# UnchartedWhispers/Distributed-Data-Parallel-Experiment

Measured on AMD Instinct MI355X. Metric: samples_per_sec_whole_node, higher is better.
Workload: dtype bf16

## Files before the change

csrc/include/ddpx_pipe.h:

```cpp
#pragma once

#include "ddpx_common.h"

namespace ddpx {
namespace pipe {

enum Epi : int {
  EPI_F32 = 0,
  EPI_BF16 = 1,
  EPI_BIAS_BF16 = 2,
  EPI_BIAS_RELU_BF16 = 3,
  EPI_BIAS_F32 = 4,
  EPI_RELUMASK_BF16 = 5,
  EPI_SGD = 6,
  EPI_BNSTAT_BF16 = 7,
  EPI_BNBWD_BF16 = 8,
};

enum Mode : int { MODE_PLAIN = 0, MODE_IM2COL_FWD = 1, MODE_IM2COL_BWD = 2, MODE_IM2COL_COL = 3 };

struct FastDiv {
  unsigned magic;
  int shift;
};
// ... 41 lines not shown
  int sgd_plain;
  float* slab;
  unsigned slab_bytes;
  int* tcnt;
  void* cs_out;
  int cs_flags;
  int* cs_tcnt;
  int im_slow;
  long long* stamp;
  const unsigned short* bn_y;
  const float* bn_a;
  const float* bn_b;
  const float* bn_mean;
  const float* bn_rstd;
  int bn_pool;
};

__device__ __forceinline__ void stamp_at(const Params& p, int tid, int k) {
  if (p.stamp && tid == 0)
    p.stamp[((size_t)blockIdx.y * gridDim.x + blockIdx.x) * 8 + k] = (long long)__builtin_amdgcn_s_memrealtime();
}

constexpr unsigned kOOB = 0x80000000u;

template <int ROWB>
__device__ __forceinline__ int tr_swz(int k) {
  if constexpr (ROWB >= 256) return (k & 3) | (((k >> 3) & 1) << 2);
  else if constexpr (ROWB == 128) return ((k >> 1) & 1) | (((k >> 3) & 1) << 1);
  else return (k >> 3) & 1;
}

// ... 253 lines not shown
  } else if constexpr (E == EPI_SGD) {
    stored = v * p.alpha;
    float d = fmaf(p.sgd.wd, pv, stored);
    if (p.sgd.mom != 0.f) {
      d = fmaf(p.sgd.mom, bv, d);
      *b_out = d;
    }
    *p_out = fmaf(-lr, d, pv);
  } else {
    const bool pos = (auxv & 0x8000u) == 0 && (auxv & 0x7fffu) != 0;
    stored = pos ? bf2f(f2bf(v * p.alpha)) : 0.f;
  }
  return stored;
}

template <int E, int BM, int BN, int NT = 256>
__device__ __forceinline__ void epilogue_vec(const Params& p, void* Cbase, const float* T, int m0, int n0, int tid,
                                             float (&csum)[4]) {
  constexpr int Q = BN / 4;
  constexpr int RSTEP = NT / Q;
  constexpr int NV = BM / RSTEP;
  constexpr int TLD = BN + 4;
  const int cq = tid % Q, r0 = tid / Q;
  const int n = n0 + 4 * cq;
  const bool vec = (n + 3 < p.N) && ((p.ldc & 3) == 0);
  float lr = 0.f;
  if constexpr (E == EPI_SGD) lr = *p.sgd.lr;
  constexpr bool HAS_BIAS = E == EPI_BIAS_BF16 || E == EPI_BIAS_RELU_BF16 || E == EPI_BIAS_F32;
  float bq[4] = {0.f, 0.f, 0.f, 0.f};
  if constexpr (HAS_BIAS) {
    if (vec && !(reinterpret_cast<uintptr_t>(p.bias + n) & 15)) {
      const f32x4 b4 = *reinterpret_cast<const f32x4*>(p.bias + n);
#pragma unroll
      for (int q = 0; q < 4; ++q) bq[q] = b4[q];
    } else {
#pragma unroll
      for (int q = 0; q < 4; ++q) bq[q] = n + q < p.N ? p.bias[n + q] : 0.f;
    }
  }
  constexpr int CH = E == EPI_SGD ? (NV < 8 ? NV : 8) : (NV < 4 ? NV : 4);
#pragma unroll
  for (int i0 = 0; i0 < NV; i0 += CH) {
  f32x4 pin[CH], bin[CH], cin[CH];
  u32x2 ain[CH];
#pragma unroll
  for (int i = 0; i < CH; ++i) {
    const int m = m0 + r0 + (i0 + i) * RSTEP;
    pin[i] = bin[i] = cin[i] = (f32x4){0.f, 0.f, 0.f, 0.f};
    ain[i] = (u32x2){0u, 0u};
    if (m >= p.M) continue;
    const size_t off = (size_t)m * p.ldc + n;
    if (vec) {
      if constexpr (E == EPI_SGD) {
        if (p.sgd_plain) {
          pin[i] = *reinterpret_cast<const f32x4*>(p.sgd.p + off);
          if (p.sgd.mom != 0.f) bin[i] = *reinterpret_cast<const f32x4*>(p.sgd.buf + off);
        } else {
          pin[i] = __builtin_nontemporal_load(reinterpret_cast<const f32x4*>(p.sgd.p + off));
          if (p.sgd.mom != 0.f) bin[i] = __builtin_nontemporal_load(reinterpret_cast<const f32x4*>(p.sgd.buf + off));
// ... 217 lines not shown
  const int kend = p.klen ? min(p.K, kbeg + p.klen) : p.K;
  void* Cbase = p.C;
  if (p.klen && !SK) Cbase = reinterpret_cast<char*>(p.C) + (size_t)split * p.split_stride * (p.epi == EPI_F32 ? 4 : 2);

  const __amdgpu_buffer_rsrc_t ra = __builtin_amdgcn_make_buffer_rsrc((void*)p.A, 0, p.a_bytes, 0x00020000);
  const __amdgpu_buffer_rsrc_t rb = __builtin_amdgcn_make_buffer_rsrc((void*)p.B, 0, p.b_bytes, 0x00020000);

  f32x4 acc[FM][FN];
#pragma unroll
  for (int i = 0; i < FM; ++i)
#pragma unroll
    for (int j = 0; j < FN; ++j) acc[i][j] = (f32x4){0.f, 0.f, 0.f, 0.f};

  const int nk = (kend - kbeg + BK - 1) / BK;

  constexpr bool A_IM = AK && (AMODE == MODE_IM2COL_FWD || AMODE == MODE_IM2COL_BWD);
  ImRows<A_IM ? BM : 8 * NW, NW> arow;
  const bool a_fast = A_IM && !p.im_slow && (p.conv.C & 63) == 0;
  if constexpr (A_IM) {
    if (a_fast) im_rows_init<BM, NW>(arow, p.conv, m0, p.M, wave, lane);
  }
  constexpr bool B_COL = !BKc && BMODE == MODE_IM2COL_COL;
  ColRows<B_COL ? BN : 8 * NW, NW> bcol;
  const bool b_fast = B_COL && !p.im_slow && (64 % p.conv.W) == 0;
  if constexpr (B_COL) {
    if (b_fast) col_rows_init<BN, NW>(bcol, p.conv, n0, p.N, wave, lane);
  }

  auto issue = [&](int t) {
    char* slot = smem + (t % STAGES) * SLOT;
// ... 55 lines not shown
      }
      for (int j = nk > D ? nk - D : 0; j < nk; ++j) {
        wait_vmcnt_rt((nk - 1 - j) * LPL);
        lds_signal(ring_full + j % STAGES, lane);
      }
      return;
    }
    for (int t = 0; t < nk; ++t) {
      const int sl = t % STAGES;
      lds_wait_ge(ring_full + sl, (t / STAGES + 1) * LW);
      mma_slot(t);
      asm volatile("s_waitcnt lgkmcnt(0)" ::: "memory");
      lds_signal(ring_free + sl, lane);
    }
  } else {
#pragma unroll
  for (int s = 0; s < STAGES - 1; ++s)
    if (s < nk) issue(s);

  for (int t = 0; t < nk; ++t) {
    const int ahead = min(STAGES - 2, nk - 1 - t);
    if (STAGES >= 6 && ahead >= 4) wait_vmcnt<(STAGES >= 6 ? 4 : 0) * LPW>();
    else if (STAGES >= 5 && ahead >= 3) wait_vmcnt<(STAGES >= 5 ? 3 : 0) * LPW>();
    else if (ahead >= 2) wait_vmcnt<2 * LPW>();
    else if (ahead == 1) wait_vmcnt<LPW>();
    else wait_vmcnt<0>();
    __builtin_amdgcn_s_barrier();
    asm volatile("" ::: "memory");
    if (t + STAGES - 1 < nk) issue(t + STAGES - 1);
    mma_slot(t);
// ... 30 lines not shown
        for (int j = 0; j < FN; ++j)
          v[i][j] = __builtin_bit_cast(f32x4, __builtin_amdgcn_raw_buffer_load_b128(rsl, slab_off(sp, i * FN + j), 0,
                                                                                    16 ));
#pragma unroll
      for (int i = 0; i < FM; ++i)
#pragma unroll
        for (int j = 0; j < FN; ++j) acc[i][j] = sp == 0 ? v[i][j] : acc[i][j] + v[i][j];
    }
    stamp_at(p, tid, 3);
  }

  constexpr int TLD = BN + 4;
  constexpr int SCR = (NT / (BN / 4) + 2) * BN * 4;
  constexpr int EH = (BM * TLD * 4 + SCR <= STAGES * SLOT) ? 1 : ((BM / 2) * TLD * 4 + SCR <= STAGES * SLOT) ? 2 : 4;
  static_assert(WGM % EH == 0, "epilogue parts must align with wave rows");
  constexpr int BMH = BM / EH;
  constexpr int WPH = WGM / EH;
  float* T = reinterpret_cast<float*>(smem);
  static_assert(BMH * TLD * 4 + SCR <= STAGES * SLOT, "epilogue LDS overflow");
  float* red = T + BMH * TLD;
  float* colres = red + (NT / (BN / 4)) * BN;
  float cs[4] = {0.f, 0.f, 0.f, 0.f};
  float st_n = 0.f, st_mean = 0.f, st_m2 = 0.f;
#pragma unroll
  for (int h = 0; h < EH; ++h) {
    if (h == 0) __builtin_amdgcn_s_barrier();
    else __syncthreads();
    if (wm / WPH == h) {
      const int mr = (wm % WPH) * (BM / WGM) + 4 * (lane >> 4);
      const int nc = wn * (BN / 2) + (lane & 15);
// ... 23 lines not shown
        if constexpr (LW == 0 && AMODE == MODE_IM2COL_BWD &&
                      ((NW == 8 && BM == 256 && BN == 128 && STAGES == 3) ||
                       (NW == 8 && BM == 128 && BN == 128 && STAGES != 3))) {
          float s2[4] = {0.f, 0.f, 0.f, 0.f};
          epilogue_bnbwd<BMH, BN, NT>(p, Cbase, T, mh, n0, tid, ch, s2);
          __syncthreads();
          quad_colsum<BN, NT>(red, ch, tid, colres);
          const size_t st = (size_t)tm * EH + h;
          if (tid < BN && n0 + tid < p.N) p.colsum[(st * 2) * p.N + n0 + tid] = colres[tid];
          quad_colsum<BN, NT>(red, s2, tid, colres);
          if (tid < BN && n0 + tid < p.N) p.colsum[(st * 2 + 1) * p.N + n0 + tid] = colres[tid];
#pragma unroll
          for (int q = 0; q < 4; ++q) ch[q] = 0.f;
        }
        break;
      default: epilogue_vec<EPI_RELUMASK_BF16, BMH, BN, NT>(p, Cbase, T, mh, n0, tid, ch); break;
    }
#pragma unroll
    for (int q = 0; q < 4; ++q) cs[q] += ch[q];
    if (LW == 0 && p.colsum && p.epi == EPI_BNSTAT_BF16) {
      __syncthreads();
      quad_colsum<BN, NT>(red, ch, tid, colres);
      const int rows_valid = min(BMH, p.M - mh);
      float* tmean = colres + BN;
      if (tid < BN) tmean[tid] = rows_valid > 0 ? colres[tid] / (float)rows_valid : 0.f;
      __syncthreads();
      {
        constexpr int Q = BN / 4, RSTEP = NT / Q, NV = BMH / RSTEP;
        const int cq = tid % Q, r0 = tid / Q;
        float m2[4] = {0.f, 0.f, 0.f, 0.f};
#pragma unroll
// ... 67 lines not shown
      v[q] = __uint_as_float(__builtin_amdgcn_raw_buffer_load_b32(
          rcs, (unsigned)(((size_t)(t0 + q) * p.N + n0 + tid) * 4), 0, 16 ));
#pragma unroll
    for (int q = 0; q < 8; ++q) tot += v[q];
  }
  const int n = n0 + tid;
  if (p.sgd.p) {
    sgd_apply_pre(p.sgd, n, tot, lrv, pv, mv);
  } else if (p.cs_flags & 1) {
    unsigned short* o = reinterpret_cast<unsigned short*>(p.cs_out) + n;
    *o = f2bf((p.cs_flags & 2) ? tot + bf2f(*o) : tot);
  } else {
    float* o = reinterpret_cast<float*>(p.cs_out) + n;
    *o = (p.cs_flags & 2) ? tot + *o : tot;
  }
}

template <int BM, int BN, int STAGES, bool AK, bool BKc, int AMODE, int BMODE, int NW = 4, int KSUB = 1,
          bool SK = false, int LW = 0>
static hipError_t launch(const Params& p, int splits, hipStream_t s) {
  const int tiles = ((p.M + BM - 1) / BM) * ((p.N + BN - 1) / BN);
  hipLaunchKernelGGL((gemm_pipe_kernel<BM, BN, STAGES, AK, BKc, AMODE, BMODE, NW, KSUB, SK, LW>),
                     dim3(tiles, splits), dim3((NW + LW) * 64), 0, s, p);
  return hipGetLastError();
}

constexpr int kNumCfgs = 26;
static inline bool eight_wave(int cfg) {
  return cfg == 8 || cfg == 13 || cfg == 14 || cfg == 15 || cfg == 22 || cfg == 25;
}
// ... 79 lines not shown
```

csrc/include/ddpx_wgrad_sgd.h:

```cpp
#pragma once

#include <cstdlib>

#include "ddpx_mx.h"
#include "ddpx_pipe.h"

namespace ddpx {
namespace wsgd {

constexpr int BN = 128;
constexpr int NK = 8;
constexpr int kStampSlots = 256;

template <int BM, int STAGES>
struct Cfg {
  static_assert(BM == 64 || BM == 128, "tile height");
  static_assert(STAGES == 3 || (STAGES == 4 && BM == 64), "ring depth");
  static constexpr int A_SUB = BM * 64 * 2, B_SUB = BN * 64 * 2, SLOT = A_SUB + B_SUB;
  static constexpr bool SBUF = BM == 128;
  static constexpr int ALD = (STAGES >= 4 || SBUF) ? BN : BN + 4;
  static constexpr int ACC_BYTES = BM * ALD * 4;
  static constexpr int LDS_BYTES = STAGES * SLOT + (SBUF ? 1 : 2) * ACC_BYTES;
  static_assert(LDS_BYTES <= 160 * 1024, "LDS");
  __host__ __device__ static constexpr int tile_col(int row, int col) {
    return SBUF ? (col ^ (((row >> 2) & 3) << 4)) : col;
  }
};

template <int BM, int STAGES, bool FP8, int NSW, bool NORD, int NMW, int PROBE = 0>
__global__ void __launch_bounds__(64 * NMW + 64 * NSW) wgrad_sgd_ws_kernel(pipe::Params p0, pipe::Params p1, int nt1) {
  using C = Cfg<BM, STAGES>;
  constexpr int ALD = C::ALD, ACC_BYTES = C::ACC_BYTES, LDS_BYTES = C::LDS_BYTES;
  constexpr int A_SUB = C::A_SUB, SLOT = C::SLOT;
  constexpr bool SBUF = C::SBUF;
  static_assert(NMW == 4 || NMW == 8, "math waves");
  static_assert(BM == 64 || (NMW == 8 && !FP8), "the 128-row tile: 8 math waves, no MX-FP8 copy");
  static_assert(PROBE == 0 || PROBE == 3 || PROBE == 4, "probe");
  constexpr int WN = NMW / 2;
  constexpr int WMR = BM / 2;
  constexpr int FM = WMR / 16, FN = BN / WN / 16;
  constexpr int LPW = (BM + BN) / (8 * NMW);
  __shared__ __attribute__((aligned(1024))) char smem[LDS_BYTES];
  float* const accb = reinterpret_cast<float*>(smem + STAGES * SLOT);

  const int tid = threadIdx.x;
// ... 215 lines not shown
      const float inv = ldexpf(1.f, -e);
      const unsigned lo = mx::quant4(v[0], v[1], v[2], v[3], inv, mx::kMaxE4M3, false);
      const unsigned hi = mx::quant4(v[4], v[5], v[6], v[7], inv, mx::kMaxE4M3, false);
      const int Mg = sel ? p1.M : p0.M;
      *reinterpret_cast<u32x2*>(qd + (size_t)(n0 + c) * Mg + m0 + 32 * b + 8 * sub) = (u32x2){lo, hi};
      unsigned char* const ed = sel ? ET1 : ET0;
      if (sub == 0 && ed) {
        if (b == 0) {
          qt_e0 = (unsigned)(e + 127);
        } else {
          *reinterpret_cast<unsigned short*>(ed + (size_t)(n0 + c) * (Mg / 32) + m0 / 32) =
              (unsigned short)(qt_e0 | ((unsigned)(e + 127) << 8));
        }
      }
    };
#pragma unroll
    for (int v = 0; v < DIST; ++v)
      if constexpr (PROBE != 3) load_vec(0, v, rp[v], rm[v]);
    for (int t = 0; t < nk; ++t) {
      mark();
      __builtin_amdgcn_s_barrier();
    }
    mark();
    __builtin_amdgcn_s_barrier();
    constexpr int TPI = SV / DIST;
    f32x4 gq[UPK];
    auto read_ahead = [&](int v0) {
      if constexpr (SBUF && PROBE != 3) {
#pragma unroll
        for (int k = 0; k < UPK; ++k) gq[k] = grad_vec(accb, v0 + k);
// ... 88 lines not shown
  Variant v;
  v.bm = 64;
  v.stages = (env_stages == 3 || env_stages == 4) ? env_stages : (large ? 4 : 3);
  v.fp8 = fp8;
  v.nsw = qt ? 8 : (env_nsw == 4 || env_nsw == 8) ? env_nsw : (large ? 8 : 4);
  v.nord = env_nord;
  v.nmw = (env_nmw != 4 && v.nsw == 4 && v.nord) ? 8 : 4;
  const bool can128 = m128 && !fp8 && !qt && env_stages != 4 && env_nsw != 8 && env_nmw != 4 && env_nord;
  const bool want128 = env_tile == 128 || (env_tile != 64 && ntiles >= 2LL * num_cus);
  if (want128 && can128) v.bm = 128, v.stages = 3, v.nsw = 4, v.nmw = 8;
  const bool toy = !fp8 && v.stages == 3 && v.nsw == 4 && v.nord;
  v.probe = (toy && (env_probe == 3 || env_probe == 4)) ? env_probe : 0;
  return v;
}

using Kernel = void (*)(pipe::Params, pipe::Params, int);

template <int STAGES, bool FP8>
static inline Kernel layout_kernel(const Variant& v) {
  if (v.nmw == 8) return wgrad_sgd_ws_kernel<64, STAGES, FP8, 4, true, 8>;
  if (v.nsw == 8) return v.nord ? wgrad_sgd_ws_kernel<64, STAGES, FP8, 8, true, 4>
                                : wgrad_sgd_ws_kernel<64, STAGES, FP8, 8, false, 4>;
  return v.nord ? wgrad_sgd_ws_kernel<64, STAGES, FP8, 4, true, 4> : wgrad_sgd_ws_kernel<64, STAGES, FP8, 4, false, 4>;
}

static inline Kernel kernel_of(const Variant& v) {
  if (v.bm == 128) {
    if (v.probe == 3) return wgrad_sgd_ws_kernel<128, 3, false, 4, true, 8, 3>;
    if (v.probe == 4) return wgrad_sgd_ws_kernel<128, 3, false, 4, true, 8, 4>;
    return wgrad_sgd_ws_kernel<128, 3, false, 4, true, 8>;
  }
  if (v.probe == 3)
    return v.nmw == 8 ? wgrad_sgd_ws_kernel<64, 3, false, 4, true, 8, 3> : wgrad_sgd_ws_kernel<64, 3, false, 4, true, 4, 3>;
  if (v.probe == 4)
    return v.nmw == 8 ? wgrad_sgd_ws_kernel<64, 3, false, 4, true, 8, 4> : wgrad_sgd_ws_kernel<64, 3, false, 4, true, 4, 4>;
  if (v.stages == 4) return v.fp8 ? layout_kernel<4, true>(v) : layout_kernel<4, false>(v);
  return v.fp8 ? layout_kernel<3, true>(v) : layout_kernel<3, false>(v);
}

static inline Variant plan(const pipe::Params& p0, const pipe::Params& p1, bool pair, bool qt, int num_cus) {
  const long long nt64 = (long long)(p0.M / 64) * (p0.N / BN) + (pair ? (long long)(p1.M / 64) * (p1.N / BN) : 0);
  const bool m128 = p0.M % 128 == 0 && (!pair || p1.M % 128 == 0);
  return select_variant(nt64, num_cus, p0.sgd.q8 != nullptr, qt, m128);
}

static inline hipError_t launch_variant(const pipe::Params& p0, const pipe::Params& p1, bool pair, bool qt,
                                        int num_cus, hipStream_t s) {
  const Variant v = plan(p0, p1, pair, qt, num_cus);
  const int nt1 = pair ? (p1.M / v.bm) * (p1.N / BN) : 0;
  const int ntiles = (p0.M / v.bm) * (p0.N / BN) + nt1;
  const int grid = ntiles < num_cus ? ntiles : num_cus;
  hipLaunchKernelGGL(kernel_of(v), dim3(grid), dim3(64 * (v.nmw + v.nsw)), 0, s, p0, p1, nt1);
  return hipGetLastError();
}

static inline hipError_t launch(const pipe::Params& p, int num_cus, hipStream_t s) {
  return launch_variant(p, p, false, false, num_cus, s);
}

static inline bool pair_compatible(const pipe::Params& a, const pipe::Params& b) {
  return a.K == b.K && a.alpha == b.alpha && a.sgd.lr == b.sgd.lr && a.sgd.mom == b.sgd.mom && a.sgd.wd == b.sgd.wd;
}

static inline hipError_t launch_pair(const pipe::Params& p0, const pipe::Params& p1, int num_cus, hipStream_t s) {
  if ((p0.sgd.q8 != nullptr) != (p1.sgd.q8 != nullptr)) return hipErrorInvalidValue;
  const bool qt = p0.sgd.q8t != nullptr || p1.sgd.q8t != nullptr;
  if (qt && !p0.sgd.q8) return hipErrorInvalidValue;
  return launch_variant(p0, p1, true, qt, num_cus, s);
}

}
}
```

csrc/kernels/gemm_pipe.hip:

```cpp
#include <cstdlib>

#include "ddpx_gemm_dispatch.h"
#include "ddpx_pipe.h"
#include "ddpx_wgrad_sgd.h"

namespace ddpx {
namespace pipe {

static int pick(int M, int N, int K, bool ak, bool bk) {
  auto tiles = [&](int bm, int bn) { return ((M + bm - 1) / bm) * ((N + bn - 1) / bn); };
  if (!ak && !bk) return tiles(64, 128) >= 512 ? 5 : 7;
  if (tiles(128, 128) >= 512 && K >= 2048) return 21;
  return 12;
}

static int plan(int M, int N, int K, bool ak, bool bk, int epi, int* cfg) {
  *cfg = pick(M, N, K, ak, bk);
  static const int sk_cfg = [] {
    const char* e = getenv("DDPX_SPLITK");
    return e ? atoi(e) : 0;
  }();
  static const int sk_max = [] {
    const char* e = getenv("DDPX_SPLITK_MAX");
    return e ? atoi(e) : 2;
// ... 57 lines not shown
  if (a_bytes >= 0x80000000ull || b_bytes >= 0x80000000ull) return -4;
  pipe::Params p{(const unsigned short*)A, (const unsigned short*)B, C, bias, (const unsigned short*)aux, colsum,
                 M, N, K, lda, ldb, ldc, ldaux, epi, accumulate, alpha, (unsigned)a_bytes, (unsigned)b_bytes,
                 SgdArgs{sgd_p, sgd_buf, (unsigned short*)sgd_shadow, sgd_lr, sgd_mom, sgd_wd},
                 pipe::make_geom(0, 0, 0, 0), 0, 0, 0, nullptr, 0u, nullptr, cs_out, cs_flags, cs_tcnt};
  p.stamp = g_stamp;
  if (cs_tcnt && (!colsum || epi == pipe::EPI_SGD || epi == pipe::EPI_BNSTAT_BF16 || (!cs_out && !sgd_p) ||
                  (sgd_p && !sgd_lr)))
    return -10;
  if (epi == pipe::EPI_SGD && (!sgd_p || !sgd_lr || (sgd_mom != 0.f && !sgd_buf))) return -5;
  static const int sgd_plain = [] {
    const char* e = getenv("DDPX_SGD_PLAIN");
    return e && e[0] == '1' ? 1 : 0;
  }();
  p.sgd_plain = sgd_plain;
  int cfg = tile_cfg >= 0 ? tile_cfg : pipe::pick(M, N, K, a_kcontig, b_kcontig);
  if (cs_tcnt && pipe::eight_wave(cfg)) return -11;
  if (cfg >= 16 && cfg <= 20 && (epi == pipe::EPI_SGD || epi == pipe::EPI_BNSTAT_BF16)) return -12;
  if (splits > 1) {
    if (epi == pipe::EPI_SGD || epi == pipe::EPI_BNSTAT_BF16 || !slab || !tcnt || tile_cfg < 0 || !a_kcontig)
      return -7;
    int bm, bn;
    pipe::tile_of(cfg, &bm, &bn);
    const long long tiles = (long long)((M + bm - 1) / bm) * ((N + bn - 1) / bn);
    if (slab_floats < (long long)splits * tiles * bm * bn || slab_floats * 4 >= 0x80000000ll) return -8;
    int klen = (K + splits - 1) / splits;
    klen = (klen + 63) / 64 * 64;
    if ((K + klen - 1) / klen != splits) return -9;
    p.klen = klen;
    p.slab = slab;
// ... 18 lines not shown
    return (int)wsgd::launch(p, cus, stream);
  }
  hipError_t e;
  if (splits > 1) {
    e = b_kcontig ? pipe::dispatch_sk_kk(p, cfg, splits, stream) : pipe::dispatch_sk_kn(p, cfg, splits, stream);
    return (int)e;
  }
  const int S = 1;
  if (a_kcontig && b_kcontig) e = pipe::dispatch_kk(p, cfg, S, stream);
  else if (a_kcontig) e = pipe::dispatch_kn(p, cfg, S, stream);
  else if (b_kcontig) e = pipe::dispatch_mk(p, cfg, S, stream);
  else e = pipe::dispatch_mn(p, cfg, S, stream);
  return (int)e;
}

DDPX_API int ddpx_wgrad_sgd_pair_t(const void* A0, const void* B0, int M0, int N0, int lda0, int ldb0, int ldc0,
                                   float* p0, float* buf0, void* sh0, void* q80, void* s80, void* q8t0, void* s8t0,
                                   const void* A1, const void* B1, int M1, int N1, int lda1, int ldb1, int ldc1,
                                   float* p1, float* buf1, void* sh1, void* q81, void* s81, void* q8t1, void* s8t1,
                                   int K, const float* lr, float mom, float wd, hipStream_t stream) {
  auto make = [&](const void* A, const void* B, int M, int N, int lda, int ldb, int ldc, float* pp, float* buf,
                  void* sh, void* q8, void* s8, void* q8t, void* s8t) {
    const size_t a_bytes = ((size_t)(K - 1) * lda + M) * 2, b_bytes = ((size_t)(K - 1) * ldb + N) * 2;
    return pipe::Params{(const unsigned short*)A, (const unsigned short*)B, pp, nullptr, nullptr, nullptr,
                        M, N, K, lda, ldb, ldc, 0, pipe::EPI_SGD, 0, 1.f, (unsigned)a_bytes, (unsigned)b_bytes,
                        SgdArgs{pp, buf, (unsigned short*)sh, lr, mom, wd, (unsigned char*)q8, (unsigned char*)s8,
                                (unsigned char*)q8t, (unsigned char*)s8t},
                        pipe::make_geom(0, 0, 0, 0), 0, 0, 0, nullptr, 0u, nullptr, nullptr, 0, nullptr};
  };
  if (K <= 0 || lda0 % 8 || ldb0 % 8 || lda1 % 8 || ldb1 % 8 || M0 % 8 || N0 % 8 || M1 % 8 || N1 % 8) return -20;
  if (((uintptr_t)A0 | (uintptr_t)B0 | (uintptr_t)A1 | (uintptr_t)B1) & 15) return -20;
  if ((q8t0 || q8t1) && (!q80 || !q81)) return -20;
  pipe::Params q0 = make(A0, B0, M0, N0, lda0, ldb0, ldc0, p0, buf0, sh0, q80, s80, q8t0, s8t0);
  const pipe::Params q1 = make(A1, B1, M1, N1, lda1, ldb1, ldc1, p1, buf1, sh1, q81, s81, q8t1, s8t1);
  q0.stamp = g_stamp;
  if ((size_t)q0.a_bytes != ((size_t)(K - 1) * lda0 + M0) * 2 || (size_t)q1.b_bytes != ((size_t)(K - 1) * ldb1 + N1) * 2)
    return -20;
  if (!wsgd::eligible(q0, false, false) || !wsgd::eligible(q1, false, false) || !wsgd::pair_compatible(q0, q1))
    return -20;
  if ((q80 != nullptr) != (q81 != nullptr)) return -20;
  int dev = 0, cus = 0;
  if (hipGetDevice(&dev) != hipSuccess ||
      hipDeviceGetAttribute(&cus, hipDeviceAttributeMultiprocessorCount, dev) != hipSuccess || cus <= 0)
    cus = 256;
  return (int)wsgd::launch_pair(q0, q1, cus, stream);
}

DDPX_API int ddpx_wgrad_sgd_pair(const void* A0, const void* B0, int M0, int N0, int lda0, int ldb0, int ldc0,
                                 float* p0, float* buf0, void* sh0, void* q80, void* s80, const void* A1,
                                 const void* B1, int M1, int N1, int lda1, int ldb1, int ldc1, float* p1, float* buf1,
                                 void* sh1, void* q81, void* s81, int K, const float* lr, float mom, float wd,
                                 hipStream_t stream) {
  return ddpx_wgrad_sgd_pair_t(A0, B0, M0, N0, lda0, ldb0, ldc0, p0, buf0, sh0, q80, s80, nullptr, nullptr, A1, B1,
                               M1, N1, lda1, ldb1, ldc1, p1, buf1, sh1, q81, s81, nullptr, nullptr, K, lr, mom, wd,
                               stream);
}

DDPX_API int ddpx_wgrad_sgd_plan(int M0, int N0, int M1, int N1, int K, int fp8, int qt, int* bm, int* stages,
                                 int* nsw, int* nmw) {
  const bool pair = M1 > 0;
// ... 19 lines not shown
```

ddpx/ops/gemm.py:

```python
from __future__ import annotations

import torch

from ..runtime import native


EPI_F32 = 0
EPI_BF16 = 1
EPI_BIAS_BF16 = 2
EPI_BIAS_RELU_BF16 = 3
EPI_BIAS_F32 = 4
EPI_RELUMASK_BF16 = 5
EPI_SGD = 6

_OUT_DTYPE = {
    EPI_F32: torch.float32,
    EPI_BF16: torch.bfloat16,
    EPI_BIAS_BF16: torch.bfloat16,
    EPI_BIAS_RELU_BF16: torch.bfloat16,
    EPI_BIAS_F32: torch.float32,
    EPI_RELUMASK_BF16: torch.bfloat16,
}


# ... 93 lines not shown
    if out_dtype == torch.bfloat16:
        epi = EPI_BIAS_RELU_BF16 if relu else (EPI_BIAS_BF16 if bias is not None else EPI_BF16)
        _req(not (relu and bias is None), "relu epilogue requires a bias")
    else:
        _req(not relu, "fp32 output epilogue has no relu")
        epi = EPI_BIAS_F32 if bias is not None else EPI_F32
    if out is None:
        out = torch.empty((M, N), dtype=_OUT_DTYPE[epi], device=x.device)
    _req(tuple(out.shape) == (M, N) and out.stride(1) == 1 and out.stride(0) % 8 == 0
         and out.data_ptr() % 16 == 0 and out.dtype == _OUT_DTYPE[epi], "bad out tensor")
    return gemm_raw(x, w, out, M=M, N=N, K=K, lda=x.stride(0), ldb=w.stride(0), ldc=out.stride(0), a_kcontig=True,
                    b_kcontig=True, epi=epi, bias=bias, tile=tile, splits=splits)


def linear_dgrad(dy, w, relu_mask_of=None, out=None, tile=-1, bias_grad=None, bias_grad_accumulate=False,
                 bias_sgd=None, splits=None):
    _check_bf16_2d(dy, "dy")
    _check_bf16_2d(w, "w")
    M, N = dy.shape
    N2, K = w.shape
    _req(N == N2, f"dy {tuple(dy.shape)} incompatible with w {tuple(w.shape)}")
    epi = EPI_BF16
    if relu_mask_of is not None:
        _check_bf16_2d(relu_mask_of, "relu_mask_of")
        _req(tuple(relu_mask_of.shape) == (M, K), "mask shape must equal dX shape")
        epi = EPI_RELUMASK_BF16
    if out is None:
        out = torch.empty((M, K), dtype=torch.bfloat16, device=dy.device)
    _req(out.shape == (M, K) and out.is_contiguous() and out.dtype == torch.bfloat16, "bad out tensor")
    part = None
    if bias_grad is not None or bias_sgd is not None:
        _req(bias_grad is None or (bias_grad.numel() == K and bias_grad.is_contiguous()),
             "bias_grad must be contiguous [K]")
        _req(bias_sgd is None or bias_sgd[0].numel() == K, "bias_sgd target must have K elements")
        T = tiles_m(M, K, N, True, False, tile)
        part = torch.empty((T, K), dtype=torch.float32, device=dy.device)
    in_launch = tile not in _EIGHT_WAVE_TILES
    _req(in_launch or bias_sgd is None, "fused bias SGD needs a 4-wave dgrad tile")
    gemm_raw(dy, w, out, M=M, N=K, K=N, lda=dy.stride(0), ldb=w.stride(0), ldc=K, a_kcontig=True,
             b_kcontig=False, epi=epi, aux=relu_mask_of,
             ldaux=(relu_mask_of.stride(0) if relu_mask_of is not None else 0), tile=tile, colsum=part,
             splits=splits,
             cs_out=bias_grad if in_launch else None, cs_accumulate=bias_grad_accumulate,
             cs_sgd=bias_sgd if in_launch else None)
    if part is not None and not in_launch and bias_grad is not None:
        s = part.sum(0).to(bias_grad.dtype)
        bias_grad.add_(s) if bias_grad_accumulate else bias_grad.copy_(s)
    return out


_EIGHT_WAVE_TILES = (8, 13, 14, 15, 22, 25)

# ... 32 lines not shown


native.register_kernel_sig("ddpx_wgrad_sgd_pair", native.c_int, *([native.c_void_p, native.c_void_p] + [native.c_int] * 5
                                                                  + [native.c_void_p] * 5) * 2,
                           native.c_int, native.c_void_p, native.c_float, native.c_float, native.c_void_p)


native.register_kernel_sig("ddpx_wgrad_sgd_pair_t", native.c_int, *([native.c_void_p, native.c_void_p] + [native.c_int] * 5
                                                                    + [native.c_void_p] * 7) * 2,
                           native.c_int, native.c_void_p, native.c_float, native.c_float, native.c_void_p)


native.register_kernel_sig("ddpx_wgrad_sgd_plan", native.c_int, *([native.c_int] * 7 + [native.c_void_p] * 4))


def wgrad_sgd_plan(M0, N0, M1=0, N1=0, K=512, fp8=False, transposed=False):
    import ctypes
    out = [ctypes.c_int(0) for _ in range(4)]
    rc = native.kernels().ddpx_wgrad_sgd_plan(int(M0), int(N0), int(M1), int(N1), int(K), int(bool(fp8)),
                                              int(bool(transposed)), *[ctypes.addressof(o) for o in out])
    if rc == -20:
        return None
    native.check(rc, "ddpx_wgrad_sgd_plan")
    return dict(zip(("bm", "stages", "nsw", "nmw"), (o.value for o in out)))


def wgrad_sgd_pair(dy0, x0, sgd0, dy1, x1, sgd1, mx0=None, mx1=None, mxt0=None, mxt1=None) -> bool:
    for t, n in ((dy0, "dy0"), (x0, "x0"), (dy1, "dy1"), (x1, "x1")):
        _check_bf16_2d(t, n)
    if dy0.shape[0] != dy1.shape[0] or x0.shape[0] != dy0.shape[0] or x1.shape[0] != dy1.shape[0]:
        return False
    if sgd0[3] is not sgd1[3] or sgd0[4] != sgd1[4] or sgd0[5] != sgd1[5]:
        return False
    K = dy0.shape[0]
    transposed = mxt0 is not None or mxt1 is not None
    if transposed and (mx0 is None or mx1 is None):
        return False
    args = []
    for dy, x, sg, mx, mxt in ((dy0, x0, sgd0, mx0, mxt0), (dy1, x1, sgd1, mx1, mxt1)):
        M, N = dy.shape[1], x.shape[1]
        _req(sg[0].numel() == M * N, "sgd target size mismatch")
        if mx is not None:
            _req(mx[0].dtype == torch.uint8 and mx[0].numel() == M * N and mx[0].is_contiguous()
                 and mx[1].dtype == torch.uint8 and mx[1].numel() == M * N // 32 and N % 32 == 0,
                 "fp8 copy must be uint8 [M, N] codes + [M, N/32] scales")
        if mxt is not None:
            _req(mxt[0].dtype == torch.uint8 and tuple(mxt[0].shape) == (N, M) and mxt[0].is_contiguous()
                 and mxt[1].dtype == torch.uint8 and tuple(mxt[1].shape) == (N, M // 32) and mxt[1].is_contiguous()
                 and M % 64 == 0, "transposed fp8 copy must be uint8 [N, M] codes + [N, M/32] scales, M % 64 == 0")
        args += [dy.data_ptr(), x.data_ptr(), M, N, dy.stride(0), x.stride(0), N, sg[0].data_ptr(),
                 native.ptr(sg[1]), native.ptr(sg[2]), native.ptr(mx[0] if mx else None),
                 native.ptr(mx[1] if mx else None)]
        if transposed:
            args += [native.ptr(mxt[0] if mxt else None), native.ptr(mxt[1] if mxt else None)]
    lr = sg[3]
    fn = native.kernels().ddpx_wgrad_sgd_pair_t if transposed else native.kernels().ddpx_wgrad_sgd_pair
    rc = fn(*args, K, lr.data_ptr(), float(sgd0[4]), float(sgd0[5]), native.stream_handle())
    if rc == -20:
        return False
    native.check(rc, "ddpx_wgrad_sgd_pair")
    return True
```

ddpx/ops/mlp.py:

```python
from __future__ import annotations

import os

import torch

from . import gemm as G
from ..optim.sgd import take_lr_advance
from .head import head_backward, head_forward

_PAIR_WGRAD = os.environ.get("DDPX_WGRAD_PAIR", "1") != "0"
_FP8_WGRAD = os.environ.get("DDPX_FP8_WGRAD", "0") == "1"
_FP8_DGRAD = os.environ.get("DDPX_FP8_DGRAD", "0") == "1"


def _dgrad_mx8(dpre, wq, h, bias_grad=None, bias_acc=False, bias_sgd=None):
    from . import fp8 as F8
    from .elementwise import colsum_bf16, sgd_flat_
    dq = F8.quant(dpre, F8.E4M3)
    dx = F8.gemm(dq, wq, epi=G.EPI_RELUMASK_BF16, aux=h)
    if bias_sgd is not None:
        p, buf, sh, lr, mom, wd = bias_sgd
        g = torch.empty(p.numel(), dtype=torch.float32, device=dx.device)
        colsum_bf16(dx, g)
        sgd_flat_(p, buf if buf is not None else torch.zeros_like(p), g, sh, lr, mom, wd)
    elif bias_grad is not None:
        if bias_grad.dtype == torch.float32:
            colsum_bf16(dx, bias_grad, accumulate=bias_acc)
# ... 81 lines not shown
    ps = _params(model)
    L = len(ps) - 1
    wl, bl = ps[-1]
    bprev = ps[L - 1][1]
    fused = flat.fused_spec(wl) is not None
    fp8_dgrad = _FP8_DGRAD and bool(getattr(model, "fp8", False)) and hs[L].is_cuda
    if fp8_dgrad and flat.shadow8t is None and not torch.cuda.is_current_stream_capturing():
        flat.enable_fp8_transposed()
    dpre = torch.empty_like(hs[L])
    if fused:
        head_backward(dl, grad_out, hs[L], flat.shadow_of(wl), None, None, dH=dpre, relu_mask=True,
                      sgd_w=flat.fused_spec(wl), sgd_b=flat.fused_spec(bl), sgd_prev=flat.fused_spec(bprev))
        for p in (wl, bl, bprev):
            flat.mark_updated(p)
        deferred = None
        for l in range(L - 1, -1, -1):
            w, _ = ps[l]
            dnext = None
            if l > 0:
                bp = ps[l - 1][1]
                if fp8_dgrad:
                    dnext = _dgrad_mx8(dpre, flat.mx8t_weight(w), hs[l], bias_sgd=flat.fused_spec(bp))
                else:
                    dnext = G.linear_dgrad(dpre, flat.shadow_of(w), relu_mask_of=hs[l], bias_sgd=flat.fused_spec(bp))
                flat.mark_updated(bp)
            if l == 1 and not saved8 and _PAIR_WGRAD:
                deferred = (dpre, hs[1], flat.fused_spec(w), w)
            elif l == 0 and deferred is not None:
                d1, h1, s1, w1 = deferred
                s0 = flat.fused_spec(w)
                emit = flat.shadow8 is not None and flat.fp8_from_optimizer
                mx1, mx0 = (flat.mx8_views(w1), flat.mx8_views(w)) if emit else (None, None)
                if mx1 is None or mx0 is None:
                    mx1 = mx0 = None
                mxt1 = flat.mx8t_views(w1) if (fp8_dgrad and mx1 is not None) else None
                paired = G.wgrad_sgd_pair(d1, h1, s1, dpre, hs[0], s0, mx1, mx0, mxt1, None)
                if not paired:
                    G.linear_wgrad(d1, h1, None, sgd=s1)
                    _wgrad(saved8, 0, dpre, hs[0], None, sgd=s0)
                flat.mark_updated(w1, fp8_written=paired and mx1 is not None,
                                  fp8t_written=paired and mxt1 is not None)
                flat.mark_updated(w, fp8_written=paired and mx0 is not None)
                dpre = dnext
                continue
            else:
                _wgrad(saved8, l, dpre, hs[l], None, sgd=flat.fused_spec(w))
            flat.mark_updated(w)
            dpre = dnext
        return
    dW, acc = flat.grad_target(wl)
    db, accb = flat.grad_target(bl)
    dbp, accp = flat.grad_target(bprev)
# ... 84 lines not shown
```

Before: 2.465 million.

## Defer dgrad bias colsum-SGD into paired wgrad kernel and prefetch relu mask

The layer-1 dgrad no longer finishes its bias column-sum and SGD update inside its own launch. It writes per-tile partials, and the paired wgrad+SGD kernel reduces them and applies the bias update in its producer warps, with a standalone finish kernel as fallback. Separately, the 64x64 two-stage plain GEMM tile now issues the relu-mask aux loads for the epilogue before the main K loop so their latency overlaps compute. This is meant to remove a serialized in-launch finish step and hide epilogue load latency, at the cost of extra registers and more work placed in the wgrad kernel.

```diff
diff --git a/csrc/include/ddpx_pipe.h b/csrc/include/ddpx_pipe.h
--- a/csrc/include/ddpx_pipe.h
+++ b/csrc/include/ddpx_pipe.h
@@ -79,7 +79,18 @@
   const float* bn_mean;
   const float* bn_rstd;
   int bn_pool;
+  int epi_pf;
 };
+
+struct EpiPre {
+  u32x4 lo, hi;
+};
+
+template <int BM, int BN, int STAGES, int AMODE, int BMODE, int NW, int KSUB, bool SK, int LW>
+constexpr bool epi_prefetch_tile() {
+  return BM == 64 && BN == 64 && STAGES == 2 && NW == 4 && KSUB == 2 && !SK && LW == 0 && AMODE == MODE_PLAIN &&
+         BMODE == MODE_PLAIN;
+}
 
 __device__ __forceinline__ void stamp_at(const Params& p, int tid, int k) {
   if (p.stamp && tid == 0)
@@ -363,9 +374,33 @@
   return stored;
 }
 
-template <int E, int BM, int BN, int NT = 256>
+template <int BM, int BN, int NT>
+__device__ __forceinline__ EpiPre epi_prefetch(const Params& p, int m0, int n0, int tid) {
+  constexpr int Q = BN / 4, RSTEP = NT / Q, NV = BM / RSTEP;
+  static_assert(NV <= 4, "the prefetch holds one chunk of 4 vectors");
+  const int cq = tid % Q, r0 = tid / Q;
+  const int n = n0 + 4 * cq;
+  const bool vec = (n + 3 < p.N) && ((p.ldc & 3) == 0);
+  EpiPre pre{(u32x4){0u, 0u, 0u, 0u}, (u32x4){0u, 0u, 0u, 0u}};
+  if (p.epi == EPI_RELUMASK_BF16) {
+    if (vec) {
+      u32x2 a[4] = {{0u, 0u}, {0u, 0u}, {0u, 0u}, {0u, 0u}};
+#pragma unroll
+      for (int i = 0; i < NV; ++i) {
+        const int m = m0 + r0 + i * RSTEP;
+        a[i] = *reinterpret_cast<const u32x2*>(p.aux + (m < p.M ? (size_t)m * p.ldaux : (size_t)0) + n);
+      }
+      pre.lo = (u32x4){a[0][0], a[0][1], a[1][0], a[1][1]};
+      pre.hi = (u32x4){a[2][0], a[2][1], a[3][0], a[3][1]};
+    }
+  }
+  return pre;
+}
+
+template <int E, int BM, int BN, int NT = 256, bool PF = false>
 __device__ __forceinline__ void epilogue_vec(const Params& p, void* Cbase, const float* T, int m0, int n0, int tid,
-                                             float (&csum)[4]) {
+                                             float (&csum)[4], const EpiPre pre = EpiPre{},
+                                             bool use_pre = false) {
   constexpr int Q = BN / 4;
   constexpr int RSTEP = NT / Q;
   constexpr int NV = BM / RSTEP;
@@ -392,6 +427,19 @@
   for (int i0 = 0; i0 < NV; i0 += CH) {
   f32x4 pin[CH], bin[CH], cin[CH];
   u32x2 ain[CH];
+  bool loaded = false;
+  if constexpr (PF && E == EPI_RELUMASK_BF16) {
+    if (use_pre && i0 == 0) {
+      loaded = true;
+#pragma unroll
+      for (int i = 0; i < CH; ++i) {
+        pin[i] = bin[i] = cin[i] = (f32x4){0.f, 0.f, 0.f, 0.f};
+        const u32x4 h = i < 2 ? pre.lo : pre.hi;
+        ain[i] = (i & 1) ? (u32x2){h[2], h[3]} : (u32x2){h[0], h[1]};
+      }
+    }
+  }
+  if (!loaded)
 #pragma unroll
   for (int i = 0; i < CH; ++i) {
     const int m = m0 + r0 + (i0 + i) * RSTEP;
@@ -639,6 +687,10 @@
 
   const int nk = (kend - kbeg + BK - 1) / BK;
 
+  constexpr bool PF = epi_prefetch_tile<BM, BN, STAGES, AMODE, BMODE, NW, KSUB, SK, LW>();
+  EpiPre epf{(u32x4){0u, 0u, 0u, 0u}, (u32x4){0u, 0u, 0u, 0u}};
+  const bool use_pre = PF && p.epi_pf;
+
   constexpr bool A_IM = AK && (AMODE == MODE_IM2COL_FWD || AMODE == MODE_IM2COL_BWD);
   ImRows<A_IM ? BM : 8 * NW, NW> arow;
   const bool a_fast = A_IM && !p.im_slow && (p.conv.C & 63) == 0;
@@ -724,6 +776,9 @@
       lds_signal(ring_free + sl, lane);
     }
   } else {
+  if constexpr (PF) {
+    if (use_pre) epf = epi_prefetch<BM, BN, NT>(p, m0, n0, tid);
+  }
 #pragma unroll
   for (int s = 0; s < STAGES - 1; ++s)
     if (s < nk) issue(s);
@@ -784,6 +839,7 @@
   constexpr int SCR = (NT / (BN / 4) + 2) * BN * 4;
   constexpr int EH = (BM * TLD * 4 + SCR <= STAGES * SLOT) ? 1 : ((BM / 2) * TLD * 4 + SCR <= STAGES * SLOT) ? 2 : 4;
   static_assert(WGM % EH == 0, "epilogue parts must align with wave rows");
+  static_assert(!PF || EH == 1, "the prefetched chunk is the first chunk of the whole tile");
   constexpr int BMH = BM / EH;
   constexpr int WPH = WGM / EH;
   float* T = reinterpret_cast<float*>(smem);
@@ -837,7 +893,7 @@
           for (int q = 0; q < 4; ++q) ch[q] = 0.f;
         }
         break;
-      default: epilogue_vec<EPI_RELUMASK_BF16, BMH, BN, NT>(p, Cbase, T, mh, n0, tid, ch); break;
+      default: epilogue_vec<EPI_RELUMASK_BF16, BMH, BN, NT, PF>(p, Cbase, T, mh, n0, tid, ch, epf, use_pre); break;
     }
 #pragma unroll
     for (int q = 0; q < 4; ++q) cs[q] += ch[q];
@@ -935,6 +991,37 @@
     float* o = reinterpret_cast<float*>(p.cs_out) + n;
     *o = (p.cs_flags & 2) ? tot + *o : tot;
   }
+}
+
+struct ColFinish {
+  const float* part;
+  int tiles_m, n;
+  SgdArgs sgd;
+};
+
+__device__ __forceinline__ void colsum_finish_col(const ColFinish& cf, int n) {
+  const __amdgpu_buffer_rsrc_t rcs = __builtin_amdgcn_make_buffer_rsrc(
+      (void*)cf.part, 0, (unsigned)((size_t)cf.tiles_m * cf.n * 4), 0x00020000);
+  const float pv = __builtin_nontemporal_load(cf.sgd.p + n);
+  float mv = 0.f;
+  if (cf.sgd.mom != 0.f) mv = __builtin_nontemporal_load(cf.sgd.buf + n);
+  const float lrv = *cf.sgd.lr;
+  float tot = 0.f;
+  for (int t0 = 0; t0 < cf.tiles_m; t0 += 8) {
+    float v[8];
+#pragma unroll
+    for (int q = 0; q < 8; ++q)
+      v[q] = __uint_as_float(
+          __builtin_amdgcn_raw_buffer_load_b32(rcs, (unsigned)(((size_t)(t0 + q) * cf.n + n) * 4), 0, 0));
+#pragma unroll
+    for (int q = 0; q < 8; ++q) tot += v[q];
+  }
+  sgd_apply_pre(cf.sgd, n, tot, lrv, pv, mv);
+}
+
+static inline bool colfinish_ok(const ColFinish& cf) {
+  return cf.part && cf.tiles_m > 0 && cf.n > 0 && (size_t)cf.tiles_m * cf.n * 4 < 0x80000000ull && cf.sgd.p &&
+         cf.sgd.lr && (cf.sgd.mom == 0.f || cf.sgd.buf);
 }
 
 template <int BM, int BN, int STAGES, bool AK, bool BKc, int AMODE, int BMODE, int NW = 4, int KSUB = 1,
diff --git a/csrc/include/ddpx_wgrad_sgd.h b/csrc/include/ddpx_wgrad_sgd.h
--- a/csrc/include/ddpx_wgrad_sgd.h
+++ b/csrc/include/ddpx_wgrad_sgd.h
@@ -28,7 +28,8 @@
 };
 
 template <int BM, int STAGES, bool FP8, int NSW, bool NORD, int NMW, int PROBE = 0>
-__global__ void __launch_bounds__(64 * NMW + 64 * NSW) wgrad_sgd_ws_kernel(pipe::Params p0, pipe::Params p1, int nt1) {
+__global__ void __launch_bounds__(64 * NMW + 64 * NSW)
+wgrad_sgd_ws_kernel(pipe::Params p0, pipe::Params p1, int nt1, pipe::ColFinish cf) {
   using C = Cfg<BM, STAGES>;
   constexpr int ALD = C::ALD, ACC_BYTES = C::ACC_BYTES, LDS_BYTES = C::LDS_BYTES;
   constexpr int A_SUB = C::A_SUB, SLOT = C::SLOT;
@@ -274,6 +275,10 @@
         }
       }
     };
+    if (cf.part) {
+      for (int c0 = 16 * (int)blockIdx.x; c0 < cf.n; c0 += 16 * (int)gridDim.x)
+        if (st < 16 && c0 + st < cf.n) pipe::colsum_finish_col(cf, c0 + st);
+    }
 #pragma unroll
     for (int v = 0; v < DIST; ++v)
       if constexpr (PROBE != 3) load_vec(0, v, rp[v], rm[v]);
@@ -392,7 +397,7 @@
   return v;
 }
 
-using Kernel = void (*)(pipe::Params, pipe::Params, int);
+using Kernel = void (*)(pipe::Params, pipe::Params, int, pipe::ColFinish);
 
 template <int STAGES, bool FP8>
 static inline Kernel layout_kernel(const Variant& v) {
@@ -423,12 +428,12 @@
 }
 
 static inline hipError_t launch_variant(const pipe::Params& p0, const pipe::Params& p1, bool pair, bool qt,
-                                        int num_cus, hipStream_t s) {
+                                        int num_cus, hipStream_t s, const pipe::ColFinish& cf = pipe::ColFinish{}) {
   const Variant v = plan(p0, p1, pair, qt, num_cus);
   const int nt1 = pair ? (p1.M / v.bm) * (p1.N / BN) : 0;
   const int ntiles = (p0.M / v.bm) * (p0.N / BN) + nt1;
   const int grid = ntiles < num_cus ? ntiles : num_cus;
-  hipLaunchKernelGGL(kernel_of(v), dim3(grid), dim3(64 * (v.nmw + v.nsw)), 0, s, p0, p1, nt1);
+  hipLaunchKernelGGL(kernel_of(v), dim3(grid), dim3(64 * (v.nmw + v.nsw)), 0, s, p0, p1, nt1, cf);
   return hipGetLastError();
 }
 
@@ -440,12 +445,13 @@
   return a.K == b.K && a.alpha == b.alpha && a.sgd.lr == b.sgd.lr && a.sgd.mom == b.sgd.mom && a.sgd.wd == b.sgd.wd;
 }
 
-static inline hipError_t launch_pair(const pipe::Params& p0, const pipe::Params& p1, int num_cus, hipStream_t s) {
+static inline hipError_t launch_pair(const pipe::Params& p0, const pipe::Params& p1, int num_cus, hipStream_t s,
+                                     const pipe::ColFinish& cf = pipe::ColFinish{}) {
   if ((p0.sgd.q8 != nullptr) != (p1.sgd.q8 != nullptr)) return hipErrorInvalidValue;
   const bool qt = p0.sgd.q8t != nullptr || p1.sgd.q8t != nullptr;
   if (qt && !p0.sgd.q8) return hipErrorInvalidValue;
-  return launch_variant(p0, p1, true, qt, num_cus, s);
-}
-
-}
-}
+  return launch_variant(p0, p1, true, qt, num_cus, s, cf);
+}
+
+}
+}
diff --git a/csrc/kernels/gemm_pipe.hip b/csrc/kernels/gemm_pipe.hip
--- a/csrc/kernels/gemm_pipe.hip
+++ b/csrc/kernels/gemm_pipe.hip
@@ -95,6 +95,11 @@
     return e && e[0] == '1' ? 1 : 0;
   }();
   p.sgd_plain = sgd_plain;
+  static const int epi_pf = [] {
+    const char* e = getenv("DDPX_EPI_PREFETCH");
+    return e && e[0] == '0' ? 0 : 1;
+  }();
+  p.epi_pf = epi_pf;
   int cfg = tile_cfg >= 0 ? tile_cfg : pipe::pick(M, N, K, a_kcontig, b_kcontig);
   if (cs_tcnt && pipe::eight_wave(cfg)) return -11;
   if (cfg >= 16 && cfg <= 20 && (epi == pipe::EPI_SGD || epi == pipe::EPI_BNSTAT_BF16)) return -12;
@@ -143,11 +148,12 @@
   return (int)e;
 }
 
-DDPX_API int ddpx_wgrad_sgd_pair_t(const void* A0, const void* B0, int M0, int N0, int lda0, int ldb0, int ldc0,
-                                   float* p0, float* buf0, void* sh0, void* q80, void* s80, void* q8t0, void* s8t0,
-                                   const void* A1, const void* B1, int M1, int N1, int lda1, int ldb1, int ldc1,
-                                   float* p1, float* buf1, void* sh1, void* q81, void* s81, void* q8t1, void* s8t1,
-                                   int K, const float* lr, float mom, float wd, hipStream_t stream) {
+static int wgrad_sgd_pair_impl(const void* A0, const void* B0, int M0, int N0, int lda0, int ldb0, int ldc0,
+                               float* p0, float* buf0, void* sh0, void* q80, void* s80, void* q8t0, void* s8t0,
+                               const void* A1, const void* B1, int M1, int N1, int lda1, int ldb1, int ldc1,
+                               float* p1, float* buf1, void* sh1, void* q81, void* s81, void* q8t1, void* s8t1,
+                               int K, const float* lr, float mom, float wd, const pipe::ColFinish& cf,
+                               hipStream_t stream) {
   auto make = [&](const void* A, const void* B, int M, int N, int lda, int ldb, int ldc, float* pp, float* buf,
                   void* sh, void* q8, void* s8, void* q8t, void* s8t) {
     const size_t a_bytes = ((size_t)(K - 1) * lda + M) * 2, b_bytes = ((size_t)(K - 1) * ldb + N) * 2;
@@ -172,7 +178,43 @@
   if (hipGetDevice(&dev) != hipSuccess ||
       hipDeviceGetAttribute(&cus, hipDeviceAttributeMultiprocessorCount, dev) != hipSuccess || cus <= 0)
     cus = 256;
-  return (int)wsgd::launch_pair(q0, q1, cus, stream);
+  return (int)wsgd::launch_pair(q0, q1, cus, stream, cf);
+}
+
+DDPX_API int ddpx_wgrad_sgd_pair_t(const void* A0, const void* B0, int M0, int N0, int lda0, int ldb0, int ldc0,
+                                   float* p0, float* buf0, void* sh0, void* q80, void* s80, void* q8t0, void* s8t0,
+                                   const void* A1, const void* B1, int M1, int N1, int lda1, int ldb1, int ldc1,
+                                   float* p1, float* buf1, void* sh1, void* q81, void* s81, void* q8t1, void* s8t1,
+                                   int K, const float* lr, float mom, float wd, hipStream_t stream) {
+  return wgrad_sgd_pair_impl(A0, B0, M0, N0, lda0, ldb0, ldc0, p0, buf0, sh0, q80, s80, q8t0, s8t0, A1, B1, M1, N1,
+                             lda1, ldb1, ldc1, p1, buf1, sh1, q81, s81, q8t1, s8t1, K, lr, mom, wd, pipe::ColFinish{},
+                             stream);
+}
+
+DDPX_API int ddpx_wgrad_sgd_pair_cs(const void* A0, const void* B0, int M0, int N0, int lda0, int ldb0, int ldc0,
+                                    float* p0, float* buf0, void* sh0, void* q80, void* s80, void* q8t0, void* s8t0,
+                                    const void* A1, const void* B1, int M1, int N1, int lda1, int ldb1, int ldc1,
+                                    float* p1, float* buf1, void* sh1, void* q81, void* s81, void* q8t1, void* s8t1,
+                                    int K, const float* lr, float mom, float wd, const float* cs_part, int cs_tiles_m,
+                                    int cs_n, float* cs_p, float* cs_buf, void* cs_sh, const float* cs_lr, float cs_mom,
+                                    float cs_wd, hipStream_t stream) {
+  const pipe::ColFinish cf{cs_part, cs_tiles_m, cs_n, SgdArgs{cs_p, cs_buf, (unsigned short*)cs_sh, cs_lr, cs_mom, cs_wd}};
+  if (!pipe::colfinish_ok(cf)) return -21;
+  return wgrad_sgd_pair_impl(A0, B0, M0, N0, lda0, ldb0, ldc0, p0, buf0, sh0, q80, s80, q8t0, s8t0, A1, B1, M1, N1,
+                             lda1, ldb1, ldc1, p1, buf1, sh1, q81, s81, q8t1, s8t1, K, lr, mom, wd, cf, stream);
+}
+
+__global__ void __launch_bounds__(64) dgrad_colsum_finish_kernel(pipe::ColFinish cf) {
+  const int n = blockIdx.x * 64 + threadIdx.x;
+  if (n < cf.n) pipe::colsum_finish_col(cf, n);
+}
+
+DDPX_API int ddpx_dgrad_colsum_finish(const float* cs_part, int cs_tiles_m, int cs_n, float* cs_p, float* cs_buf,
+                                void* cs_sh, const float* cs_lr, float cs_mom, float cs_wd, hipStream_t stream) {
+  const pipe::ColFinish cf{cs_part, cs_tiles_m, cs_n, SgdArgs{cs_p, cs_buf, (unsigned short*)cs_sh, cs_lr, cs_mom, cs_wd}};
+  if (!pipe::colfinish_ok(cf)) return -21;
+  hipLaunchKernelGGL(dgrad_colsum_finish_kernel, dim3((cs_n + 63) / 64), dim3(64), 0, stream, cf);
+  return (int)hipGetLastError();
 }
 
 DDPX_API int ddpx_wgrad_sgd_pair(const void* A0, const void* B0, int M0, int N0, int lda0, int ldb0, int ldc0,
diff --git a/ddpx/ops/gemm.py b/ddpx/ops/gemm.py
--- a/ddpx/ops/gemm.py
+++ b/ddpx/ops/gemm.py
@@ -131,7 +131,7 @@
 
 
 def linear_dgrad(dy, w, relu_mask_of=None, out=None, tile=-1, bias_grad=None, bias_grad_accumulate=False,
-                 bias_sgd=None, splits=None):
+                 bias_sgd=None, splits=None, defer_finish=False):
     _check_bf16_2d(dy, "dy")
     _check_bf16_2d(w, "w")
     M, N = dy.shape
@@ -153,6 +153,13 @@
         T = tiles_m(M, K, N, True, False, tile)
         part = torch.empty((T, K), dtype=torch.float32, device=dy.device)
     in_launch = tile not in _EIGHT_WAVE_TILES
+    if defer_finish:
+        _req(bias_sgd is not None and bias_grad is None, "defer_finish needs bias_sgd (and no bias_grad)")
+        gemm_raw(dy, w, out, M=M, N=K, K=N, lda=dy.stride(0), ldb=w.stride(0), ldc=K, a_kcontig=True,
+                 b_kcontig=False, epi=epi, aux=relu_mask_of,
+                 ldaux=(relu_mask_of.stride(0) if relu_mask_of is not None else 0), tile=tile, colsum=part,
+                 splits=splits)
+        return out, (part, bias_sgd)
     _req(in_launch or bias_sgd is None, "fused bias SGD needs a 4-wave dgrad tile")
     gemm_raw(dy, w, out, M=M, N=K, K=N, lda=dy.stride(0), ldb=w.stride(0), ldc=K, a_kcontig=True,
              b_kcontig=False, epi=epi, aux=relu_mask_of,
@@ -215,6 +222,28 @@
 native.register_kernel_sig("ddpx_wgrad_sgd_plan", native.c_int, *([native.c_int] * 7 + [native.c_void_p] * 4))
 
 
+_CS_ARGS = (native.c_void_p, native.c_int, native.c_int, native.c_void_p, native.c_void_p, native.c_void_p,
+            native.c_void_p, native.c_float, native.c_float)
+
+native.register_kernel_sig("ddpx_wgrad_sgd_pair_cs", native.c_int, *([native.c_void_p, native.c_void_p] + [native.c_int] * 5
+                                                                     + [native.c_void_p] * 7) * 2,
+                           native.c_int, native.c_void_p, native.c_float, native.c_float, *_CS_ARGS, native.c_void_p)
+
+native.register_kernel_sig("ddpx_dgrad_colsum_finish", native.c_int, *_CS_ARGS, native.c_void_p)
+
+
+def _finish_args(pending):
+    part, sgd = pending
+    _req(part.dtype == torch.float32 and part.dim() == 2 and part.is_contiguous(), "partials must be fp32 [T, N]")
+    _req(sgd[0].numel() == part.shape[1], "finish target must have one element per column")
+    return (part.data_ptr(), part.shape[0], part.shape[1], *native.sgd_args(sgd))
+
+
+def colsum_finish(pending, stream=None):
+    rc = native.kernels().ddpx_dgrad_colsum_finish(*_finish_args(pending), native.stream_handle(stream))
+    native.check(rc, "ddpx_dgrad_colsum_finish")
+
+
 def wgrad_sgd_plan(M0, N0, M1=0, N1=0, K=512, fp8=False, transposed=False):
     import ctypes
     out = [ctypes.c_int(0) for _ in range(4)]
@@ -226,7 +255,7 @@
     return dict(zip(("bm", "stages", "nsw", "nmw"), (o.value for o in out)))
 
 
-def wgrad_sgd_pair(dy0, x0, sgd0, dy1, x1, sgd1, mx0=None, mx1=None, mxt0=None, mxt1=None) -> bool:
+def wgrad_sgd_pair(dy0, x0, sgd0, dy1, x1, sgd1, mx0=None, mx1=None, mxt0=None, mxt1=None, finish=None) -> bool:
     for t, n in ((dy0, "dy0"), (x0, "x0"), (dy1, "dy1"), (x1, "x1")):
         _check_bf16_2d(t, n)
     if dy0.shape[0] != dy1.shape[0] or x0.shape[0] != dy0.shape[0] or x1.shape[0] != dy1.shape[0]:
@@ -252,9 +281,16 @@
         args += [dy.data_ptr(), x.data_ptr(), M, N, dy.stride(0), x.stride(0), N, sg[0].data_ptr(),
                  native.ptr(sg[1]), native.ptr(sg[2]), native.ptr(mx[0] if mx else None),
                  native.ptr(mx[1] if mx else None)]
-        if transposed:
+        if transposed or finish is not None:
             args += [native.ptr(mxt[0] if mxt else None), native.ptr(mxt[1] if mxt else None)]
     lr = sg[3]
+    if finish is not None:
+        rc = native.kernels().ddpx_wgrad_sgd_pair_cs(*args, K, lr.data_ptr(), float(sgd0[4]), float(sgd0[5]),
+                                                     *_finish_args(finish), native.stream_handle())
+        if rc == -20:
+            return False
+        native.check(rc, "ddpx_wgrad_sgd_pair_cs")
+        return True
     fn = native.kernels().ddpx_wgrad_sgd_pair_t if transposed else native.kernels().ddpx_wgrad_sgd_pair
     rc = fn(*args, K, lr.data_ptr(), float(sgd0[4]), float(sgd0[5]), native.stream_handle())
     if rc == -20:
diff --git a/ddpx/ops/mlp.py b/ddpx/ops/mlp.py
--- a/ddpx/ops/mlp.py
+++ b/ddpx/ops/mlp.py
@@ -11,6 +11,7 @@
 _PAIR_WGRAD = os.environ.get("DDPX_WGRAD_PAIR", "1") != "0"
 _FP8_WGRAD = os.environ.get("DDPX_FP8_WGRAD", "0") == "1"
 _FP8_DGRAD = os.environ.get("DDPX_FP8_DGRAD", "0") == "1"
+_DGRAD_FINISH_PAIR = os.environ.get("DDPX_DGRAD_FINISH", "pair") != "launch"
 
 
 def _dgrad_mx8(dpre, wq, h, bias_grad=None, bias_acc=False, bias_sgd=None):
@@ -122,6 +123,7 @@
         for p in (wl, bl, bprev):
             flat.mark_updated(p)
         deferred = None
+        pending = None
         for l in range(L - 1, -1, -1):
             w, _ = ps[l]
             dnext = None
@@ -129,6 +131,9 @@
                 bp = ps[l - 1][1]
                 if fp8_dgrad:
                     dnext = _dgrad_mx8(dpre, flat.mx8t_weight(w), hs[l], bias_sgd=flat.fused_spec(bp))
+                elif l == 1 and not saved8 and _PAIR_WGRAD and _DGRAD_FINISH_PAIR:
+                    dnext, pending = G.linear_dgrad(dpre, flat.shadow_of(w), relu_mask_of=hs[l],
+                                                    bias_sgd=flat.fused_spec(bp), defer_finish=True)
                 else:
                     dnext = G.linear_dgrad(dpre, flat.shadow_of(w), relu_mask_of=hs[l], bias_sgd=flat.fused_spec(bp))
                 flat.mark_updated(bp)
@@ -142,8 +147,10 @@
                 if mx1 is None or mx0 is None:
                     mx1 = mx0 = None
                 mxt1 = flat.mx8t_views(w1) if (fp8_dgrad and mx1 is not None) else None
-                paired = G.wgrad_sgd_pair(d1, h1, s1, dpre, hs[0], s0, mx1, mx0, mxt1, None)
+                paired = G.wgrad_sgd_pair(d1, h1, s1, dpre, hs[0], s0, mx1, mx0, mxt1, None, finish=pending)
                 if not paired:
+                    if pending is not None:
+                        G.colsum_finish(pending)
                     G.linear_wgrad(d1, h1, None, sgd=s1)
                     _wgrad(saved8, 0, dpre, hs[0], None, sgd=s0)
                 flat.mark_updated(w1, fp8_written=paired and mx1 is not None,
```

Result: no change. 2.483 million, median of 6 (+0.7%).
